# Lukeasargen/Show-Attend-and-Tell-Pytorch-Lightning

Hardware: AMD Instinct MI355X
Metric: captions/sec (train step) at B=128, 256px, seq_len=22 (higher is better)
Workload: dtype bf16; 1 GPU; C2: resnet50 encoder_size=7 encoder_dim=512 vocab=6400 T=22, 128 images/GPU x R=5 captions, trainable encoder, Adam, full lengths, decoder_tf=always; global_batch_images=128, parallelism=dp1, grad_bucket_dtype=fp32

## Files before the change

### show-attend-and-tell-pytorch-lightning_amd/csrc/api.hip

```cpp
#include <stdarg.h>

#include "../../include/sat_hip.h"
#include "decoder.h"
#include "decoder_step.h"
#include "gemm.h"
#include "gemm_bf16_common.h"
#include "temperature.h"
#include "caption_score.h"

namespace sat {
static thread_local char g_err[512] = {0};
int& dev_switch(int which) {
    static int v[SW_COUNT] = {0 , getenv("SAT_NO_WGRAD3X3") ? !atoi(getenv("SAT_NO_WGRAD3X3")) : 1,
                              getenv("SAT_REDUCE_Z16") ? atoi(getenv("SAT_REDUCE_Z16")) : 1, getenv("SAT_WIDE_TILES") ? atoi(getenv("SAT_WIDE_TILES")) : 0,
                              getenv("SAT_BN_ONEPASS") ? atoi(getenv("SAT_BN_ONEPASS")) : 1,
                              getenv("SAT_BN_VPT") ? atoi(getenv("SAT_BN_VPT")) : 2,
                              getenv("SAT_ACC_PREFETCH") ? atoi(getenv("SAT_ACC_PREFETCH")) : 0};
    return v[which];
}
int& trace_launches() { static int on = getenv("SAT_TRACE_LAUNCH") ? 1 : 0; return on; }
char* last_error_buf() { return g_err; }
int fail(int code, const char* fmt, ...) {
    va_list ap; va_start(ap, fmt); vsnprintf(g_err, sizeof g_err, fmt, ap); va_end(ap);
    return code;
}
}

using namespace sat;

extern "C" {

int sat_abi_version(void) { return SAT_HIP_ABI_VERSION; }
int sat_debug_trace_launches(int32_t on) { sat::trace_launches() = on ? 1 : 0; return SAT_OK; }
int sat_debug_option(const char* name, int32_t value) {
    if (!name) return fail(SAT_EINVAL, "debug_option: null name");
    if (!strcmp(name, "wgrad3x3")) { dev_switch(SW_WGRAD3X3) = value; return SAT_OK; }
    if (!strcmp(name, "reduce_z16")) { dev_switch(SW_REDUCE_Z16) = value; return SAT_OK; }
    if (!strcmp(name, "acc_prefetch")) { dev_switch(SW_ACC_PREFETCH) = value; return SAT_OK; }
    if (!strcmp(name, "bn_vpt")) { dev_switch(SW_BN_VPT) = value; return SAT_OK; }
    if (!strcmp(name, "bn_onepass")) { dev_switch(SW_BN_ONEPASS) = value; return SAT_OK; }
    if (!strcmp(name, "wide_tiles")) { dev_switch(SW_WIDE_TILES) = value; return SAT_OK; }
    if (!strcmp(name, "glds_tile")) { glds_force_tile() = value; return SAT_OK; }
    if (!strcmp(name, "glds_stages8")) { glds_stages8() = value; return SAT_OK; }
    if (!strcmp(name, "glds_tall_k")) { glds_tall_k() = value; return SAT_OK; }
    if (!strcmp(name, "glds_tall_conv")) { glds_tall_conv() = value; return SAT_OK; }
    if (!strcmp(name, "tile_override")) { gemm_tile_override() = value; return SAT_OK; }
    return fail(SAT_EINVAL, "debug_option: unknown option %s", name);
}
const char* sat_last_error(void) { return last_error_buf(); }

static int gemm_from_desc(const sat_gemm_desc* d, const sat_gemm_types* t, void* stream);
int sat_gemm_f32(const sat_gemm_desc* d, void* stream) { return gemm_from_desc(d, nullptr, stream); }
int sat_gemm_ex(const sat_gemm_desc* d, const sat_gemm_types* t, void* stream) {
    if (!t) return fail(SAT_EINVAL, "sat_gemm_ex: null type descriptor");
    return gemm_from_desc(d, t, stream);
}
static int gemm_from_desc(const sat_gemm_desc* d, const sat_gemm_types* t, void* stream) {
    if (!d) return fail(SAT_EINVAL, "sat_gemm_f32: null descriptor");
    if (d->amode != A_ROW && d->amode != A_KMAJOR) return fail(SAT_EINVAL, "sat_gemm_f32: amode %d (dense modes only)", d->amode);
    if (d->bmode != B_ROW && d->bmode != B_KMAJOR) return fail(SAT_EINVAL, "sat_gemm_f32: bmode %d (dense modes only)", d->bmode);
    GemmArgs g;
    g.A = d->A; g.lda = d->lda; g.a_rows = d->a_rows; g.B = d->B; g.ldb = d->ldb; g.C = d->C; g.ldc = d->ldc; g.c_rows = d->c_rows;
    g.M = d->M; g.N = d->N; g.K = d->K; g.amode = d->amode; g.bmode = d->bmode; g.accumulate = d->accumulate; g.epi = d->epi;
    g.bias = d->bias; g.e0 = d->e0; g.lde0 = d->lde0; g.c0 = d->c0; g.c1 = d->c1; g.slab = d->slab; g.slab_elems = d->slab_elems;
    if (t) { g.a_bf16 = t->a_bf16; g.b_bf16 = t->b_bf16; g.c_bf16 = t->c_bf16; g.bf16_mfma = t->bf16_mfma; }
    return launch_gemm(g, (hipStream_t)stream);
}

size_t sat_decoder_workspace_bytes(const sat_decoder_dims* d) {
    if (check_dims(d) != SAT_OK) return 0;
    return decoder_workspace_bytes(*d);
}

size_t sat_decoder_workspace_bytes_ln(const sat_decoder_dims* d, const sat_decoder_params* w) {
    if (check_dims(d) != SAT_OK) return 0;
    return decoder_workspace_bytes(*d, w && ln_on(*w));
}

static int check_params(const sat_decoder_dims* d, const sat_decoder_params* w, const char* what) {
    if (!w) return fail(SAT_EINVAL, "%s: null parameter struct", what);
    if (!w->embedding || !w->init_f_w || !w->init_f_b || !w->init_i_w || !w->init_i_b || !w->w_ih || !w->w_hh || !w->b_ih || !w->b_hh ||
        !w->att_enc || !w->att_dec || !w->att_f || !w->beta_w || !w->beta_b || !w->out_hidden || !w->out_w)
        return fail(SAT_EINVAL, "%s: null tensor in parameter struct", what);
    if (d->deep_output && !w->out_context) return fail(SAT_EINVAL, "%s: deep output needs output.context.weight", what);
    for (int l = 1; l < d->layers; ++l)
        if (!w->up_w_ih[l - 1] || !w->up_w_hh[l - 1] || !w->up_b_ih[l - 1] || !w->up_b_hh[l - 1])
            return fail(SAT_EINVAL, "%s: null tensor for LSTM layer %d", what, l);
    int ln_set = 0;
    for (int l = 0; l < d->layers; ++l) ln_set += (w->ln_gate_w[l] != nullptr) + (w->ln_gate_b[l] != nullptr) + (w->ln_cell_w[l] != nullptr) + (w->ln_cell_b[l] != nullptr);
    if (ln_set != 0 && ln_set != 4 * d->layers)
        return fail(SAT_EINVAL, "%s: %d of the %d layer-norm tensors (ln_gate_w / ln_gate_b / ln_cell_w / ln_cell_b of %d layers) are set: all or none", what, ln_set,
                    4 * d->layers, d->layers);
    return SAT_OK;
}
static int check_batch(const sat_decoder_batch* b) {
// ... 648 lines not shown
```

### show-attend-and-tell-pytorch-lightning_amd/csrc/gemm_bf16_common.h

```cpp
#pragma once
#include <stdlib.h>

#include "gemm.h"

namespace sat {

typedef __bf16 bf16x8 __attribute__((ext_vector_type(8)));
typedef __bf16 bf16x4 __attribute__((ext_vector_type(4)));
typedef short s16x4 __attribute__((ext_vector_type(4)));
typedef float f32x16 __attribute__((ext_vector_type(16)));

constexpr int NT = 256;

struct BArgs {
    const void* A; long lda; const int* a_rows;
    const void* B; long ldb;
    void* C; long ldc; const int* c_rows;
    int M, N, K;
    int accumulate, epi;
    const float* bias; const float* e0; long lde0; int c0, c1;
    ConvGeom g;
    int kchunk, nsplit;
    float* slab;
    int wide_store;
// ... 423 lines not shown
}

template <typename TC>
__global__ __launch_bounds__(256) void splitk_reduce_z16_kernel(BArgs a) {
    __shared__ float4 part[16][16];
    const int ev = threadIdx.x & 15, zl = threadIdx.x >> 4;
    const long idx4 = (long)blockIdx.x * 16 + ev;
    const long total4 = (long)a.M * a.N / 4;
    float4 v = make_float4(0.f, 0.f, 0.f, 0.f);
    if (idx4 < total4) {
        const float4* s4 = reinterpret_cast<const float4*>(a.slab);
#pragma unroll 4
        for (int z = zl; z < a.nsplit; z += 16) { const float4 t = s4[(long)z * total4 + idx4]; v.x += t.x; v.y += t.y; v.z += t.z; v.w += t.w; }
    }
    part[zl][ev] = v;
    __syncthreads();
    if (zl != 0 || idx4 >= total4) return;
#pragma unroll
    for (int l = 1; l < 16; ++l) { const float4 t = part[l][ev]; v.x += t.x; v.y += t.y; v.z += t.z; v.w += t.w; }
    const long e = idx4 * 4; const int row = (int)(e / a.N), col = (int)(e % a.N);
    if (sizeof(TC) == 4 && a.wide_store && !a.g.cls) {
        float* dst = reinterpret_cast<float*>(a.C) + (long)row * a.ldc + col;
        if (a.accumulate) { const float4 old = *reinterpret_cast<const float4*>(dst); v.x += old.x; v.y += old.y; v.z += old.z; v.w += old.w; }
        if (a.epi != EPI_NONE) { v.x = ep_value(a, row, col, v.x); v.y = ep_value(a, row, col + 1, v.y); v.z = ep_value(a, row, col + 2, v.z); v.w = ep_value(a, row, col + 3, v.w); }
        *reinterpret_cast<float4*>(dst) = v;
    } else {
        put<TC>(a, row, col, v.x); put<TC>(a, row, col + 1, v.y); put<TC>(a, row, col + 2, v.z); put<TC>(a, row, col + 3, v.w);
    }
}

template <typename TC>
inline int launch_splitk_reduce(const BArgs& k, hipStream_t st) {
    const long total = (long)k.M * k.N;
    const int z16 = dev_switch(SW_REDUCE_Z16);
    if (k.wide_slab && z16 && k.nsplit >= 32 && total / 4 / 256 < 256)
        hipLaunchKernelGGL(splitk_reduce_z16_kernel<TC>, dim3(cdiv(total / 4, 16)), dim3(256), 0, st, k);
    else if (k.wide_slab) hipLaunchKernelGGL(splitk_reduce_b4_kernel<TC>, dim3(cdiv(total / 4, 256)), dim3(256), 0, st, k);
    else hipLaunchKernelGGL(splitk_reduce_b_kernel<TC>, dim3(cdiv(total, 256)), dim3(256), 0, st, k);
    return launch_ok("splitk_reduce_b");
}

__device__ __forceinline__ void xcd_tile(int& bx, int& by, int& bz, int y_fastest = 0) {
    const unsigned total = gridDim.x * gridDim.y * gridDim.z;
    const unsigned orig = (blockIdx.z * gridDim.y + blockIdx.y) * gridDim.x + blockIdx.x;
    const unsigned q = total >> 3, r = total & 7, xcd = orig & 7, idx = orig >> 3;
    const unsigned lin = (xcd < r ? xcd * (q + 1) : r * (q + 1) + (xcd - r) * q) + idx;
    if (y_fastest) { by = lin % gridDim.y; const unsigned t2 = lin / gridDim.y; bx = t2 % gridDim.x; bz = t2 / gridDim.x; }
    else { bx = lin % gridDim.x; const unsigned t2 = lin / gridDim.x; by = t2 % gridDim.y; bz = t2 / gridDim.y; }
}

int launch_gemm_glds(const BArgs& k, int amode, int bmode, int c_bf16, int BMt, hipStream_t st, int* bm_used = nullptr);
int& glds_force_tile();
int& glds_stages8();
int& glds_tall_k();
int& glds_tall_conv();
int& glds_ablate();
int& gemm_tile_override();

}
```

### show-attend-and-tell-pytorch-lightning_amd/csrc/gemm_glds.hip

```cpp
#include <stdlib.h>

#include "gemm_bf16_common.h"

namespace sat {

template <int AM, int BMo, typename TC> int glds_run_64(const BArgs& k, hipStream_t st);
template <int AM, int BMo, typename TC> int glds_run_128(const BArgs& k, hipStream_t st);
template <int AM, int BMo, typename TC> int glds_run_128x64(const BArgs& k, hipStream_t st);
#ifdef SAT_DEV_TILES
template <int AM, int BMo, typename TC> int glds_run_256x128(const BArgs& k, hipStream_t st);
template <int AM, int BMo, typename TC> int glds_run_256(const BArgs& k, hipStream_t st);
#endif

enum { TILE_64 = 0, TILE_128 = 1, TILE_128x64 = 2, TILE_256x128 = 3, TILE_256 = 4 };
template <int AM, int BMo, typename TC>
static int rung_tiles(const BArgs& k, int tile, hipStream_t st, int* bm_used) {
    switch (tile) {
#ifdef SAT_DEV_TILES
        case TILE_256: if (bm_used) *bm_used = 256; return glds_run_256<AM, BMo, TC>(k, st);
        case TILE_256x128: if (bm_used) *bm_used = 256; return glds_run_256x128<AM, BMo, TC>(k, st);
#else
        case TILE_256: case TILE_256x128: return -1;
#endif
        case TILE_128: if (bm_used) *bm_used = 128; return glds_run_128<AM, BMo, TC>(k, st);
        case TILE_128x64: if (bm_used) *bm_used = 128; return glds_run_128x64<AM, BMo, TC>(k, st);
        default: if (bm_used) *bm_used = 64; return glds_run_64<AM, BMo, TC>(k, st);
    }
}

int& glds_force_tile() { static int v = getenv("SAT_GLDS_TILE") ? atoi(getenv("SAT_GLDS_TILE")) : -1; return v; }
int& glds_ablate() { static int v = 0; return v; }
int& glds_tall_k() { static int v = getenv("SAT_GLDS_TALL_K") ? atoi(getenv("SAT_GLDS_TALL_K")) : 1 << 30; return v; }
int& glds_tall_conv() { static int v = getenv("SAT_GLDS_TALL_CONV") ? atoi(getenv("SAT_GLDS_TALL_CONV")) : 1152; return v; }
int& glds_stages8() { static int v = getenv("SAT_GLDS_STAGES8") ? atoi(getenv("SAT_GLDS_STAGES8")) : 0; return v; }

int launch_gemm_glds(const BArgs& k0, int amode, int bmode, int c_bf16, int BMt, hipStream_t st, int* bm_used) {
    const int force_tile = glds_force_tile();
    static const int off = getenv("SAT_NO_GLDS") ? atoi(getenv("SAT_NO_GLDS")) : 0;
    static const int force_stages = getenv("SAT_GLDS_STAGES") ? atoi(getenv("SAT_GLDS_STAGES")) : 0;
    static const int deep_from = getenv("SAT_GLDS_DEEP_FROM") ? atoi(getenv("SAT_GLDS_DEEP_FROM")) : 1 << 30;
    static const int rotate = getenv("SAT_GLDS_ROT") ? atoi(getenv("SAT_GLDS_ROT")) : 1 << 20;
    if (off) return -1;
    BArgs k = k0;
    const int ktiles = cdiv(k.kchunk < k.K ? k.kchunk : k.K, 64);
    static const int s1_upto = getenv("SAT_GLDS_S1_UPTO") ? atoi(getenv("SAT_GLDS_S1_UPTO")) : 1 << 30;
    k.nstage = force_stages ? force_stages : (ktiles >= deep_from ? 4 : ((ktiles == 1 || (c_bf16 && ktiles <= s1_upto)) ? 1 : 2));
    k.rotate = rotate;
    if (k.nstage < 1) k.nstage = 1;
    if (k.nstage > 4) k.nstage = 4;
    static const int tall = getenv("SAT_GLDS_TALL") ? atoi(getenv("SAT_GLDS_TALL")) : 2;
    int tile = (BMt >= 256) ? (BMt == 256 ? TILE_256 : TILE_256x128) : (BMt == 128 ? TILE_128 : TILE_64);
    if (tile == TILE_64 && tall && bmode != B_CONV_WGRAD && k.N <= 64 && (amode == A_KMAJOR ? (tall > 1 && k.M >= 128) : k.M >= 8192)) tile = TILE_128x64;
    static const int tall_conv_tiles = getenv("SAT_GLDS_TALL_CONV_TILES") ? atoi(getenv("SAT_GLDS_TALL_CONV_TILES")) : 512;
    if (tile == TILE_128 && bmode != B_CONV_WGRAD && k.nsplit <= 1 &&
        ((amode == A_ROW && k.K <= glds_tall_k()) || ((amode == A_CONV_FWD || amode == A_CONV_DGRAD) && (k.K <= glds_tall_conv() || (long)cdiv(k.M, 128) * cdiv(k.N, 128) < tall_conv_tiles)))) tile = TILE_128x64;
    if (force_tile >= 0) tile = force_tile;
    if (tile == TILE_256 || tile == TILE_256x128) {
        const int maxs = (tile == TILE_256) ? 2 : 3;
        const int deep8 = glds_stages8();
        if (ktiles > 1) k.nstage = deep8 ? (deep8 < maxs ? deep8 : maxs) : (ktiles >= 3 ? maxs : 2);
    }
    {
        static const int order = getenv("SAT_TILE_ORDER") ? atoi(getenv("SAT_TILE_ORDER")) : -1;
        const int tbm = (tile == TILE_64) ? 64 : 128, tbn = (tile == TILE_128) ? 128 : 64;
        const int mt = cdiv(k.M, tbm), nt = cdiv(k.N, tbn);
        k.y_fastest = order >= 0 ? order : (amode == A_ROW && bmode != B_CONV_WGRAD && mt <= 16 && nt >= 2 * mt);
    }
    const ConvGeom& g = k.g;
    if (g.sw && g.sw != g.stride) return -1;
    if (k.K % 64 || k.kchunk % 64 || k.a_rows) return -1;
    if (amode == A_CONV_FWD && (g.C % 64 || g.R * g.S > 32)) return -1;
    if (amode == A_CONV_DGRAD && (g.K % 64 || g.R * g.S > 32 || (g.stride != 1 && !g.cls))) return -1;
    if (bmode == B_CONV_WGRAD && g.R * g.S > 32) return -1;
    const long lim = 1L << 30;
    long a_el = 0, b_el = 0;
    switch (amode) {
        case A_ROW: a_el = (long)k.M * k.lda; break;
        case A_KMAJOR: a_el = (long)k.K * k.lda; break;
        case A_CONV_FWD: a_el = (long)g.N * g.H * g.W * g.C; break;
        default: a_el = (long)g.N * g.P * g.Q * g.K; break;
    }
    switch (bmode) {
        case B_ROW: b_el = (long)k.N * k.ldb; break;
        case B_KMAJOR: b_el = (long)k.K * k.ldb; break;
        case B_CONV_WGRAD: b_el = (long)g.N * g.H * g.W * g.C; break;
        default: b_el = (long)g.K * g.R * g.S * g.C; break;
    }
    if (a_el >= lim || b_el >= lim) return -1;
    if ((amode == A_KMAJOR && k.M < 8) || (bmode != B_ROW && k.N < 8)) return -1;
#define SAT_GCASE(AMV, BMV, TC) return rung_tiles<AMV, BMV, TC>(k, tile, st, bm_used);
    if (amode == A_CONV_FWD && bmode == B_ROW && c_bf16) SAT_GCASE(A_CONV_FWD, B_ROW, __bf16)
    if (amode == A_ROW && bmode == B_ROW && c_bf16) SAT_GCASE(A_ROW, B_ROW, __bf16)
    if (amode == A_ROW && bmode == B_ROW && !c_bf16) SAT_GCASE(A_ROW, B_ROW, float)
    if (amode == A_CONV_DGRAD && bmode == B_CONV_DGRAD_W && c_bf16) SAT_GCASE(A_CONV_DGRAD, B_CONV_DGRAD_W, __bf16)
    if (amode == A_ROW && bmode == B_KMAJOR && c_bf16) SAT_GCASE(A_ROW, B_KMAJOR, __bf16)
    if (amode == A_ROW && bmode == B_KMAJOR && !c_bf16) SAT_GCASE(A_ROW, B_KMAJOR, float)
    if (amode == A_KMAJOR && bmode == B_CONV_WGRAD && !c_bf16) SAT_GCASE(A_KMAJOR, B_CONV_WGRAD, float)
    if (amode == A_KMAJOR && bmode == B_KMAJOR && !c_bf16) SAT_GCASE(A_KMAJOR, B_KMAJOR, float)
#undef SAT_GCASE
// ... 5 lines not shown
```

### show-attend-and-tell-pytorch-lightning_amd/csrc/gemm_glds_kernel.h

```cpp
#include <stdlib.h>

#include <initializer_list>

#pragma once
#include "gemm_bf16_common.h"
#include "profile.h"

#ifndef SAT_GLDS_ABLATE
#define SAT_GLDS_ABLATE 0
#endif

namespace sat {

typedef int i32x4 __attribute__((ext_vector_type(4)));
typedef __attribute__((address_space(3))) void* lptr_t;

__device__ void raw_buffer_load_lds(i32x4 rsrc, lptr_t lds, int size, int voffset, int soffset, int offset, int aux) __asm("llvm.amdgcn.raw.buffer.load.lds");

constexpr int OOB = (int)0x80000000;

__device__ __forceinline__ i32x4 make_rsrc(const void* base) {
    const unsigned long long b = reinterpret_cast<unsigned long long>(base);
    i32x4 r;
    r[0] = (int)(unsigned)b; r[1] = (int)(unsigned)((b >> 32) & 0xFFFF);
    r[2] = OOB;
    r[3] = 0x00020000;
    return r;
}
__device__ __forceinline__ void dma16(const i32x4& rsrc, int voff, int soff, __bf16* lds_wave_base) {
    raw_buffer_load_lds(rsrc, (lptr_t)lds_wave_base, 16, voff, soff, 0, 0);
}

__device__ __forceinline__ unsigned bit_range(int lo, int hi) {
    if (lo < 0) lo = 0;
    if (hi > 32) hi = 32;
    if (hi <= lo) return 0u;
    const unsigned upper = (hi >= 32) ? 0xFFFFFFFFu : ((1u << hi) - 1u);
    return upper & ~((1u << lo) - 1u);
}
__device__ __forceinline__ unsigned tap_mask(int rlo, int rhi, int clo, int chi, int nrow, int ncol) {
    const unsigned cm = bit_range(clo, chi < ncol ? chi : ncol);
    unsigned m = 0;
    if (rlo < 0) rlo = 0;
    if (rhi > nrow) rhi = nrow;
    for (int i = rlo; i < rhi; ++i) m |= cm << (i * ncol);
    return m;
}

template <typename T> __device__ __forceinline__ void keep_alive(const T& v) {
#if defined(__HIP_DEVICE_COMPILE__)
    asm volatile("" ::"v"(v));
#endif
}
template <typename T, typename U> __device__ __forceinline__ void keep_alive(const T& v, const U& w) { keep_alive(v); keep_alive(w); }

struct PixEnt { int off; unsigned mask; };

#ifndef SAT_GLDS_BN_PREFETCH
// ... 180 lines not shown

    f32x16 acc[TM][TN];
#pragma unroll
    for (int i = 0; i < TM; ++i)
#pragma unroll
        for (int j = 0; j < TN; ++j)
#pragma unroll
            for (int r = 0; r < 16; ++r) acc[i][j][r] = 0.f;

    constexpr bool BNS = (AM == A_CONV_DGRAD) || (AM == A_ROW && BMo == B_KMAJOR);
    constexpr bool BPF = SAT_GLDS_BN_PREFETCH;
    BnAcc<BM, BN, 64 * NW, BNS, BPF> bnacc(a, bn, tid);
    if constexpr (sizeof(TC) == 2) { bnacc.prefetch(a, bm, bn, tid); __builtin_amdgcn_sched_barrier(0); }

    int a_off[TM], a_sw[TM], b_off[TN], b_sw[TN];
#pragma unroll
    for (int i = 0; i < TM; ++i) {
        if (!AK) { const int row = wm + i * 32 + li; a_off[i] = row * KB; a_sw[i] = (row >> 1) & 7; }
        else {
            const int col = wm + i * 32 + 16 * t_mh + 4 * t_p, kr = 8 * t_h + t_q;
            const int sw = (BM >= 128) ? (kr & 3) : ((kr >> 1) & 1);
            a_off[i] = kr * BM + (((col >> 5) ^ sw) << 5) + (col & 31); a_sw[i] = 0;
        }
    }
#pragma unroll
    for (int j = 0; j < TN; ++j) {
        if (!BKM) { const int row = wn + j * 32 + li; b_off[j] = row * KB; b_sw[j] = (row >> 1) & 7; }
        else {
            const int col = wn + j * 32 + 16 * t_mh + 4 * t_p, kr = 8 * t_h + t_q;
            const int sw = (BN >= 128) ? (kr & 3) : ((kr >> 1) & 1);
            b_off[j] = kr * BN + (((col >> 5) ^ sw) << 5) + (col & 31); b_sw[j] = 0;
        }
    }

    if (kbeg < kend) {
        if (WG) {
            for (int t = 0; t < S; ++t) fill_tab(t, t);
            __syncthreads();
        }
        const int pre = (S == 1) ? 1 : S - 1;
        for (int t = 0; t < pre && t < T; ++t) issue(t, t);
        int cur = 0, nxt = S - 1;
        for (int it = 0; it < T; ++it) {
            const int ahead = (S == 1) ? 0 : min(T - 1 - it, S - 2);
            if (ahead >= 2) asm volatile("s_waitcnt vmcnt(%0)" ::"n"(2 * G) : "memory");
            else if (ahead == 1) asm volatile("s_waitcnt vmcnt(%0)" ::"n"(G) : "memory");
            else asm volatile("s_waitcnt vmcnt(0)" ::: "memory");
            asm volatile("s_waitcnt lgkmcnt(0)" ::: "memory");
            __builtin_amdgcn_s_barrier();
            asm volatile("" ::: "memory");
            const bool more = S > 1 && it + S - 1 < T;
            const __bf16* as = smem + cur * STAGE;
            const __bf16* bs = as + A_EL;
            bf16x8 af[2][TM], bf[2][TN];
            auto load_frags = [&](int kk, bf16x8 (&fa)[TM], bf16x8 (&fb)[TN]) {
#pragma unroll
                for (int i = 0; i < TM; ++i) {
                    if (!AK) fa[i] = *reinterpret_cast<const bf16x8*>(as + a_off[i] + ((((kk >> 3) + lh) ^ a_sw[i]) << 3));
                    else {
                        const __bf16* p = as + a_off[i] + kk * BM;
                        bf16x4 lo = __builtin_amdgcn_ds_read_tr16_b64_v4bf16((__attribute__((address_space(3))) bf16x4*)p);
                        bf16x4 hi = __builtin_amdgcn_ds_read_tr16_b64_v4bf16((__attribute__((address_space(3))) bf16x4*)(p + 4 * BM));
                        fa[i] = __builtin_shufflevector(lo, hi, 0, 1, 2, 3, 4, 5, 6, 7);
                    }
                }
#pragma unroll
                for (int j = 0; j < TN; ++j) {
                    if (!BKM) fb[j] = *reinterpret_cast<const bf16x8*>(bs + b_off[j] + ((((kk >> 3) + lh) ^ b_sw[j]) << 3));
                    else {
                        const __bf16* p = bs + b_off[j] + kk * BN;
                        bf16x4 lo = __builtin_amdgcn_ds_read_tr16_b64_v4bf16((__attribute__((address_space(3))) bf16x4*)p);
                        bf16x4 hi = __builtin_amdgcn_ds_read_tr16_b64_v4bf16((__attribute__((address_space(3))) bf16x4*)(p + 4 * BN));
                        fb[j] = __builtin_shufflevector(lo, hi, 0, 1, 2, 3, 4, 5, 6, 7);
                    }
                }
            };
            if (!(abl & 4) || it == 0) load_frags(0, af[0], bf[0]);
#pragma unroll
            for (int ks = 0; ks < KB / 16; ++ks) {
                if (ks + 1 < KB / 16 && (!(abl & 4) || it == 0)) load_frags((ks + 1) * 16, af[(ks + 1) & 1], bf[(ks + 1) & 1]);
                if (more) {
#pragma unroll
                    for (int jj = (ks * G) / 4; jj < ((ks + 1) * G) / 4; ++jj) issue_piece(nxt, nxt, jj);
                }
                if constexpr (!(abl & 2)) {
#pragma unroll
                    for (int i = 0; i < TM; ++i)
#pragma unroll
                        for (int j = 0; j < TN; ++j)
                            acc[i][j] = __builtin_amdgcn_mfma_f32_32x32x16_bf16(af[ks & 1][i], bf[ks & 1][j], acc[i][j], 0, 0, 0);
                } else {
#pragma unroll
                    for (int i = 0; i < TM; ++i)
#pragma unroll
                        for (int j = 0; j < TN; ++j) keep_alive(af[ks & 1][i], bf[ks & 1][j]);
                }
            }
            if (more) advance_tile();
            if (S == 1 && it + 1 < T) {
                __syncthreads();
                if (WG) { fill_tab(0, it + 1); __syncthreads(); }
                issue(0, 0);
            }
            if (WG && S > 1) fill_tab(cur, it + S);
            cur = (cur + 1 == S) ? 0 : cur + 1;
            nxt = (nxt + 1 == S) ? 0 : nxt + 1;
        }
    }
    if constexpr (abl & 8) {
#pragma unroll
        for (int i = 0; i < TM; ++i)
#pragma unroll
            for (int j = 0; j < TN; ++j) keep_alive(acc[i][j]);
        return;
    }
    if constexpr (WR == 2 && WC == 2) store_tile<BM, BN, TC, 2 * STAGE, APF, BNS, BPF>(a, acc, smem, bm, bn, bz, wm, wn, tid, lane, bnacc, sizeof(TC) == 2);
    else store_tile_w<BM, BN, WR, WC, TC, BNS, BPF>(a, acc, smem, bm, bn, bz, wm, wn, wrow, tid, lane, bnacc, sizeof(TC) == 2);
}

static const char* gname(int am, int bm) {
    if (am == A_CONV_FWD) return "conv_fwd";
    if (am == A_CONV_DGRAD) return "conv_dgrad";
    if (bm == B_CONV_WGRAD) return "conv_wgrad";
    if (am == A_ROW && bm == B_ROW) return "nt";
    if (am == A_ROW && bm == B_KMAJOR) return "nn";
    return "tn";
}

template <int BM, int BN, int WR, int WC, int AM, int BMo, typename TC>
static int rung(const BArgs& k, hipStream_t st) {
    dim3 grid(cdiv(k.N, BN), cdiv(k.M, BM), k.nsplit);
    char pname[128];
    if (profile_enabled()) {
        static const bool shapes = getenv("SAT_PROFILE_SHAPES") != nullptr;
        if (shapes) snprintf(pname, sizeof pname, "gemm_glds_%s_%dx%d M%d N%d K%d z%d", gname(AM, BMo), BM, BN, k.M, k.N, k.K, k.nsplit);
        else snprintf(pname, sizeof pname, "gemm_glds_%s_%dx%d", gname(AM, BMo), BM, BN);
    }
    ProfScope prof(pname, 2.0 * k.M * k.N * k.K, 2.0 * k.M * k.K + 2.0 * k.N * k.K + (double)sizeof(TC) * k.M * k.N, st);
    size_t lds = (size_t)k.nstage * (BM + BN) * 64 * sizeof(__bf16);
    const size_t epi_lds = (WR == 2 && WC == 2) ? ((sizeof(TC) == 2) ? (size_t)BM * (BN + 8) * 2 + 4 * BN * 2 * 4 : (size_t)(BM / 2) * (BN + 4) * 4)
                                                : store_lds_bytes<BM, BN, WR, WC, TC>();
    if (lds < epi_lds) lds = epi_lds;
    constexpr size_t LDS_DYN_MAX = 160 * 1024 - 2560;
    SAT_REQUIRE(lds <= LDS_DYN_MAX, "gemm_glds: %zu bytes of LDS for a %dx%d tile with %d stages", lds, BM, BN, k.nstage);
    static bool attr_set = false;
    if (!attr_set) {
        SAT_CHECK_HIP(hipFuncSetAttribute(reinterpret_cast<const void*>(&gemm_glds_kernel<BM, BN, WR, WC, AM, BMo, TC>), hipFuncAttributeMaxDynamicSharedMemorySize,
                                          (int)LDS_DYN_MAX));
// ... 38 lines not shown
```

### show-attend-and-tell-pytorch-lightning_amd/csrc/wgrad3x3.hip

```cpp
#include <stdlib.h>

#include "gemm_bf16_common.h"
#include "profile.h"

namespace sat {

typedef int i32x4 __attribute__((ext_vector_type(4)));
typedef __attribute__((address_space(3))) void* lptr3_t;
__device__ void raw_buffer_load_lds_w(i32x4 rsrc, lptr3_t lds, int size, int voffset, int soffset, int offset, int aux) __asm("llvm.amdgcn.raw.buffer.load.lds");

namespace {
constexpr int W3_OOB = (int)0x80000000;
constexpr int W3_WAVES = 9, W3_THREADS = 64 * W3_WAVES;
constexpr int W3_MAXP = 4;
constexpr int W3_STAGES = 3;

__device__ __forceinline__ i32x4 w3_rsrc(const void* base) {
    const unsigned long long b = reinterpret_cast<unsigned long long>(base);
    i32x4 r;
    r[0] = (int)(unsigned)b; r[1] = (int)(unsigned)((b >> 32) & 0xFFFF);
    r[2] = W3_OOB; r[3] = 0x00020000;
    return r;
}

struct W3Args {
    const __bf16* dy; const __bf16* x; float* out;
    int Nimg, H, W, C, K;
    int nr;
    int units;
    int per;
    int HP;
    int Z;
};

__global__ __launch_bounds__(W3_THREADS) void wgrad3x3_kernel(W3Args a) {
    extern __shared__ __attribute__((aligned(1024))) __bf16 smem[];
    const int tid = threadIdx.x, lane = tid & 63, wave = tid >> 6;
    const int ci0 = blockIdx.x * 64, co0 = blockIdx.y * 64, bz = blockIdx.z;
    const int W = a.W, H = a.H, C = a.C, K = a.K, nr = a.nr, HW2 = W + 2;
    const int STAGE = 64 * 64 + a.HP * 64;
    const int u0 = bz * a.per, u1 = min(a.units, u0 + a.per);
    const int upi = H / nr;
    const i32x4 rA = w3_rsrc(a.dy), rX = w3_rsrc(a.x);

    const int npieces = 8 + a.HP / 8;
    int p_off[W3_MAXP]; int p_hr[W3_MAXP]; bool p_dy[W3_MAXP], p_on[W3_MAXP], p_colok[W3_MAXP]; int p_lds[W3_MAXP];
#pragma unroll
    for (int j = 0; j < W3_MAXP; ++j) {
        const int piece = j * W3_WAVES + wave;
        p_on[j] = piece < npieces; p_dy[j] = piece < 8; p_hr[j] = 0; p_colok[j] = false; p_off[j] = 0;
        const int sl = lane & 7;
        if (p_dy[j]) {
            const int krow = piece * 8 + (lane >> 3);
            const int lq = (sl >> 2) ^ ((krow >> 1) & 1);
            p_off[j] = (krow * K + co0 + (lq * 4 + (sl & 3)) * 8) * 2;
            p_lds[j] = piece * 512;
        } else {
            const int hp = (piece - 8) * 8 + (lane >> 3);
            const int hr = hp / HW2, hc = hp - hr * HW2 - 1;
            const int lq = (sl >> 2) ^ ((hp >> 1) & 1);
            p_hr[j] = hr;
            p_colok[j] = p_on[j] && hr < nr + 2 && hc >= 0 && hc < W;
            p_off[j] = ((hr * W + hc) * C + ci0 + (lq * 4 + (sl & 3)) * 8) * 2;
            p_lds[j] = 64 * 64 + (piece - 8) * 512;
        }
    }
    auto issue = [&](int buf, int u) {
        const int n = u / upi, p0 = (u - n * upi) * nr;
        const int baseA = ((n * H + p0) * W) * K * 2;
        const int baseX = ((n * H + p0 - 1) * W) * C * 2;
        __bf16* st = smem + buf * STAGE;
#pragma unroll
        for (int j = 0; j < W3_MAXP; ++j) {
            if (!p_on[j]) continue;
            if (p_dy[j]) raw_buffer_load_lds_w(rA, (lptr3_t)(st + p_lds[j]), 16, p_off[j] + baseA, 0, 0, 0);
            else {
                const int ih = p0 - 1 + p_hr[j];
                const bool ok = p_colok[j] && ih >= 0 && ih < H;
                raw_buffer_load_lds_w(rX, (lptr3_t)(st + p_lds[j]), 16, ok ? p_off[j] + baseX : W3_OOB, 0, 0, 0);
            }
        }
    };

    const int tg = lane >> 4, ti = lane & 15;
    const int t_h = tg >> 1, t_mh = tg & 1, t_q = ti >> 2, t_p = ti & 3;
    const int tap_r = wave / 3, tap_s = wave - tap_r * 3;
    int a_off[2];
#pragma unroll
    for (int i = 0; i < 2; ++i) {
        const int col = i * 32 + 16 * t_mh + 4 * t_p, kr = 8 * t_h + t_q;
        a_off[i] = kr * 64 + (((col >> 5) ^ ((kr >> 1) & 1)) << 5) + (col & 31);
    }
    int b_off[4][2][2];
#pragma unroll
    for (int ks = 0; ks < 4; ++ks)
#pragma unroll
        for (int hf = 0; hf < 2; ++hf) {
            const int k = ks * 16 + 8 * t_h + t_q + 4 * hf;
            const int pr = k / W, q = k - pr * W;
            const int hp = (pr + tap_r) * HW2 + q + tap_s;
#pragma unroll
            for (int j = 0; j < 2; ++j) {
                const int col = j * 32 + 16 * t_mh + 4 * t_p;
                b_off[ks][hf][j] = 64 * 64 + hp * 64 + (((col >> 5) ^ ((hp >> 1) & 1)) << 5) + (col & 31);
            }
        }

    f32x16 acc[2][2];
#pragma unroll
    for (int i = 0; i < 2; ++i)
#pragma unroll
        for (int j = 0; j < 2; ++j)
#pragma unroll
            for (int r = 0; r < 16; ++r) acc[i][j][r] = 0.f;

    int mine = 0;
#pragma unroll
    for (int j = 0; j < W3_MAXP; ++j) mine += p_on[j] ? 1 : 0;
    mine = __builtin_amdgcn_readfirstlane(mine);
    if (u0 < u1) {
        issue(0, u0);
        if (u0 + 1 < u1) issue(1, u0 + 1);
        int cur = 0, nxt = 2;
        for (int u = u0; u < u1; ++u) {
            if (u + 1 < u1) {
                if (mine == 4) asm volatile("s_waitcnt vmcnt(4)" ::: "memory");
                else if (mine == 3) asm volatile("s_waitcnt vmcnt(3)" ::: "memory");
                else if (mine == 2) asm volatile("s_waitcnt vmcnt(2)" ::: "memory");
                else asm volatile("s_waitcnt vmcnt(0)" ::: "memory");
            } else asm volatile("s_waitcnt vmcnt(0)" ::: "memory");
            asm volatile("s_waitcnt lgkmcnt(0)" ::: "memory");
            __builtin_amdgcn_s_barrier();
            asm volatile("" ::: "memory");
            if (u + 2 < u1) issue(nxt, u + 2);
            const __bf16* st = smem + cur * STAGE;
#pragma unroll
            for (int ks = 0; ks < 4; ++ks) {
                bf16x8 af[2], bf[2];
#pragma unroll
                for (int i = 0; i < 2; ++i) {
                    const __bf16* p = st + a_off[i] + ks * 16 * 64;
                    bf16x4 lo = __builtin_amdgcn_ds_read_tr16_b64_v4bf16((__attribute__((address_space(3))) bf16x4*)p);
                    bf16x4 hi = __builtin_amdgcn_ds_read_tr16_b64_v4bf16((__attribute__((address_space(3))) bf16x4*)(p + 4 * 64));
                    af[i] = __builtin_shufflevector(lo, hi, 0, 1, 2, 3, 4, 5, 6, 7);
                }
#pragma unroll
                for (int j = 0; j < 2; ++j) {
                    bf16x4 lo = __builtin_amdgcn_ds_read_tr16_b64_v4bf16((__attribute__((address_space(3))) bf16x4*)(st + b_off[ks][0][j]));
                    bf16x4 hi = __builtin_amdgcn_ds_read_tr16_b64_v4bf16((__attribute__((address_space(3))) bf16x4*)(st + b_off[ks][1][j]));
                    bf[j] = __builtin_shufflevector(lo, hi, 0, 1, 2, 3, 4, 5, 6, 7);
                }
#pragma unroll
                for (int i = 0; i < 2; ++i)
#pragma unroll
                    for (int j = 0; j < 2; ++j) acc[i][j] = __builtin_amdgcn_mfma_f32_32x32x16_bf16(af[i], bf[j], acc[i][j], 0, 0, 0);
            }
            cur = (cur + 1 == W3_STAGES) ? 0 : cur + 1;
            nxt = (nxt + 1 == W3_STAGES) ? 0 : nxt + 1;
        }
    }
    const int li = lane & 31, lh = lane >> 5;
    const long N9 = 9L * C;
    float* out = a.out + (a.Z > 1 ? (long)bz * K * N9 : 0L);
#pragma unroll
    for (int i = 0; i < 2; ++i)
#pragma unroll
        for (int j = 0; j < 2; ++j)
#pragma unroll
            for (int r = 0; r < 16; ++r) {
                const int row = co0 + i * 32 + (r & 3) + 8 * (r >> 2) + 4 * lh;
                const int col = ci0 + j * 32 + li;
                out[(long)row * N9 + (long)wave * C + col] = acc[i][j][r];
            }
}
}

int wgrad3x3_eligible(const ConvGeom& g) {
    if (!dev_switch(SW_WGRAD3X3)) return 0;
    if (g.R != 3 || g.S != 3 || g.stride != 1 || g.pad != 1 || (g.sw && g.sw != 1)) return 0;
    if (g.C % 64 || g.K % 64) return 0;
    if (g.H != g.P || g.W != g.Q) return 0;
    if (!(g.W == 8 || g.W == 16 || g.W == 32 || g.W == 64)) return 0;
    if (g.H % (64 / g.W)) return 0;
    if ((long)g.N * g.H * g.W * (g.C > g.K ? g.C : g.K) >= (1L << 30)) return 0;
    return 1;
}

int launch_wgrad3x3(const void* dy, const void* x, float* dw, const ConvGeom& g, float* slab, long slab_elems, hipStream_t st) {
    W3Args a;
    a.dy = reinterpret_cast<const __bf16*>(dy); a.x = reinterpret_cast<const __bf16*>(x);
    a.Nimg = g.N; a.H = g.H; a.W = g.W; a.C = g.C; a.K = g.K;
    a.nr = 64 / g.W; a.units = g.N * (g.H / a.nr);
    a.HP = ((a.nr + 2) * (g.W + 2) + 7) / 8 * 8;
    SAT_REQUIRE(8 + a.HP / 8 <= W3_WAVES * W3_MAXP, "wgrad3x3: %d LDS-DMA pieces per k-tile", 8 + a.HP / 8);
    const long tiles = (long)(g.C / 64) * (g.K / 64), out_elems = (long)g.K * 9 * g.C;
    static const int target = getenv("SAT_W3_TARGET") ? atoi(getenv("SAT_W3_TARGET")) : 256;
    long z = target / tiles; if (z < 1) z = 1;
    if (z > a.units / 8) z = a.units / 8 > 0 ? a.units / 8 : 1;
    while (z > 1 && (!slab || z * out_elems > slab_elems)) --z;
    a.per = (int)cdiv(a.units, z); a.Z = (int)cdiv(a.units, a.per);
    a.out = a.Z > 1 ? slab : dw;
    const size_t lds = W3_STAGES * (size_t)(64 * 64 + a.HP * 64) * sizeof(__bf16);
    static bool attr_set = false;
    if (!attr_set) {
        SAT_CHECK_HIP(hipFuncSetAttribute(reinterpret_cast<const void*>(&wgrad3x3_kernel), hipFuncAttributeMaxDynamicSharedMemorySize, 128 * 1024));
        attr_set = true;
    }
    {
        char pname[128];
        if (profile_enabled()) {
            static const bool shapes = getenv("SAT_PROFILE_SHAPES") != nullptr;
            if (shapes) snprintf(pname, sizeof pname, "gemm_wgrad3x3 M%d N%d K%d z%d", g.K, 9 * g.C, g.N * g.H * g.W, a.Z);
            else snprintf(pname, sizeof pname, "gemm_wgrad3x3");
        }
        ProfScope prof(pname, 2.0 * g.K * 9.0 * g.C * g.N * g.H * g.W, 2.0 * g.N * g.H * g.W * ((double)g.C + g.K) + 4.0 * out_elems, st);
        hipLaunchKernelGGL(wgrad3x3_kernel, dim3(g.C / 64, g.K / 64, a.Z), dim3(W3_THREADS), lds, st, a);
        SAT_TRY(launch_ok("wgrad3x3_kernel"));
        if (a.Z > 1) {
            BArgs k{};
            k.M = g.K; k.N = 9 * g.C; k.C = dw; k.ldc = 9 * g.C; k.slab = slab; k.nsplit = a.Z; k.wide_store = 1; k.wide_slab = 1; k.epi = EPI_NONE;
            SAT_TRY(launch_splitk_reduce<float>(k, st));
        }
    }
    return SAT_OK;
}

}
```

Before: 32570 captions/s.

## Use inline-asm LDS fragment reads with partial lgkmcnt waits and tunable stage counts

```diff
diff --git a/show-attend-and-tell-pytorch-lightning_amd/csrc/api.hip b/show-attend-and-tell-pytorch-lightning_amd/csrc/api.hip
--- a/show-attend-and-tell-pytorch-lightning_amd/csrc/api.hip
+++ b/show-attend-and-tell-pytorch-lightning_amd/csrc/api.hip
@@ -41,6 +41,10 @@
     if (!strcmp(name, "bn_onepass")) { dev_switch(SW_BN_ONEPASS) = value; return SAT_OK; }
     if (!strcmp(name, "wide_tiles")) { dev_switch(SW_WIDE_TILES) = value; return SAT_OK; }
     if (!strcmp(name, "glds_tile")) { glds_force_tile() = value; return SAT_OK; }
+    if (!strcmp(name, "glds_stages")) { glds_force_stages() = value; return SAT_OK; }
+    if (!strcmp(name, "glds_stages_tr_bf16")) { glds_stages_tr_bf16() = value; return SAT_OK; }
+    if (!strcmp(name, "glds_stages_f32")) { glds_stages_f32() = value; return SAT_OK; }
+    if (!strcmp(name, "w3_stages")) { w3_stages() = value; return SAT_OK; }
     if (!strcmp(name, "glds_stages8")) { glds_stages8() = value; return SAT_OK; }
     if (!strcmp(name, "glds_tall_k")) { glds_tall_k() = value; return SAT_OK; }
     if (!strcmp(name, "glds_tall_conv")) { glds_tall_conv() = value; return SAT_OK; }
diff --git a/show-attend-and-tell-pytorch-lightning_amd/csrc/gemm_bf16_common.h b/show-attend-and-tell-pytorch-lightning_amd/csrc/gemm_bf16_common.h
--- a/show-attend-and-tell-pytorch-lightning_amd/csrc/gemm_bf16_common.h
+++ b/show-attend-and-tell-pytorch-lightning_amd/csrc/gemm_bf16_common.h
@@ -499,6 +499,10 @@
 int launch_gemm_glds(const BArgs& k, int amode, int bmode, int c_bf16, int BMt, hipStream_t st, int* bm_used = nullptr);
 int& glds_force_tile();
 int& glds_stages8();
+int& glds_stages_tr_bf16();
+int& glds_stages_f32();
+int& w3_stages();
+int& glds_force_stages();
 int& glds_tall_k();
 int& glds_tall_conv();
 int& glds_ablate();
diff --git a/show-attend-and-tell-pytorch-lightning_amd/csrc/gemm_glds.hip b/show-attend-and-tell-pytorch-lightning_amd/csrc/gemm_glds.hip
--- a/show-attend-and-tell-pytorch-lightning_amd/csrc/gemm_glds.hip
+++ b/show-attend-and-tell-pytorch-lightning_amd/csrc/gemm_glds.hip
@@ -30,6 +30,9 @@
 
 int& glds_force_tile() { static int v = getenv("SAT_GLDS_TILE") ? atoi(getenv("SAT_GLDS_TILE")) : -1; return v; }
 int& glds_ablate() { static int v = 0; return v; }
+int& glds_stages_tr_bf16() { static int v = getenv("SAT_GLDS_STAGES_TR_BF16") ? atoi(getenv("SAT_GLDS_STAGES_TR_BF16")) : 1; return v; }
+int& glds_stages_f32() { static int v = getenv("SAT_GLDS_STAGES_F32") ? atoi(getenv("SAT_GLDS_STAGES_F32")) : 2; return v; }
+int& glds_force_stages() { static int v = getenv("SAT_GLDS_STAGES") ? atoi(getenv("SAT_GLDS_STAGES")) : 0; return v; }
 int& glds_tall_k() { static int v = getenv("SAT_GLDS_TALL_K") ? atoi(getenv("SAT_GLDS_TALL_K")) : 1 << 30; return v; }
 int& glds_tall_conv() { static int v = getenv("SAT_GLDS_TALL_CONV") ? atoi(getenv("SAT_GLDS_TALL_CONV")) : 1152; return v; }
 int& glds_stages8() { static int v = getenv("SAT_GLDS_STAGES8") ? atoi(getenv("SAT_GLDS_STAGES8")) : 0; return v; }
@@ -37,14 +40,14 @@
 int launch_gemm_glds(const BArgs& k0, int amode, int bmode, int c_bf16, int BMt, hipStream_t st, int* bm_used) {
     const int force_tile = glds_force_tile();
     static const int off = getenv("SAT_NO_GLDS") ? atoi(getenv("SAT_NO_GLDS")) : 0;
-    static const int force_stages = getenv("SAT_GLDS_STAGES") ? atoi(getenv("SAT_GLDS_STAGES")) : 0;
+    const int force_stages = glds_force_stages();
     static const int deep_from = getenv("SAT_GLDS_DEEP_FROM") ? atoi(getenv("SAT_GLDS_DEEP_FROM")) : 1 << 30;
     static const int rotate = getenv("SAT_GLDS_ROT") ? atoi(getenv("SAT_GLDS_ROT")) : 1 << 20;
     if (off) return -1;
     BArgs k = k0;
     const int ktiles = cdiv(k.kchunk < k.K ? k.kchunk : k.K, 64);
-    static const int s1_upto = getenv("SAT_GLDS_S1_UPTO") ? atoi(getenv("SAT_GLDS_S1_UPTO")) : 1 << 30;
-    k.nstage = force_stages ? force_stages : (ktiles >= deep_from ? 4 : ((ktiles == 1 || (c_bf16 && ktiles <= s1_upto)) ? 1 : 2));
+    const int by_form = c_bf16 ? (bmode != B_ROW ? glds_stages_tr_bf16() : 1) : glds_stages_f32();
+    k.nstage = force_stages ? force_stages : (ktiles >= deep_from ? 4 : (ktiles == 1 ? 1 : by_form));
     k.rotate = rotate;
     if (k.nstage < 1) k.nstage = 1;
     if (k.nstage > 4) k.nstage = 4;
diff --git a/show-attend-and-tell-pytorch-lightning_amd/csrc/gemm_glds_kernel.h b/show-attend-and-tell-pytorch-lightning_amd/csrc/gemm_glds_kernel.h
--- a/show-attend-and-tell-pytorch-lightning_amd/csrc/gemm_glds_kernel.h
+++ b/show-attend-and-tell-pytorch-lightning_amd/csrc/gemm_glds_kernel.h
@@ -1,9 +1,11 @@
 #include <stdlib.h>
 
 #include <initializer_list>
+#include <type_traits>
 
 #pragma once
 #include "gemm_bf16_common.h"
+#include "lds_frag.h"
 #include "profile.h"
 
 #ifndef SAT_GLDS_ABLATE
@@ -290,48 +292,86 @@
             const bool more = S > 1 && it + S - 1 < T;
             const __bf16* as = smem + cur * STAGE;
             const __bf16* bs = as + A_EL;
-            bf16x8 af[2][TM], bf[2][TN];
-            auto load_frags = [&](int kk, bf16x8 (&fa)[TM], bf16x8 (&fb)[TN]) {
-#pragma unroll
-                for (int i = 0; i < TM; ++i) {
-                    if (!AK) fa[i] = *reinterpret_cast<const bf16x8*>(as + a_off[i] + ((((kk >> 3) + lh) ^ a_sw[i]) << 3));
-                    else {
-                        const __bf16* p = as + a_off[i] + kk * BM;
-                        bf16x4 lo = __builtin_amdgcn_ds_read_tr16_b64_v4bf16((__attribute__((address_space(3))) bf16x4*)p);
-                        bf16x4 hi = __builtin_amdgcn_ds_read_tr16_b64_v4bf16((__attribute__((address_space(3))) bf16x4*)(p + 4 * BM));
-                        fa[i] = __builtin_shufflevector(lo, hi, 0, 1, 2, 3, 4, 5, 6, 7);
-                    }
-                }
-#pragma unroll
-                for (int j = 0; j < TN; ++j) {
-                    if (!BKM) fb[j] = *reinterpret_cast<const bf16x8*>(bs + b_off[j] + ((((kk >> 3) + lh) ^ b_sw[j]) << 3));
-                    else {
-                        const __bf16* p = bs + b_off[j] + kk * BN;
-                        bf16x4 lo = __builtin_amdgcn_ds_read_tr16_b64_v4bf16((__attribute__((address_space(3))) bf16x4*)p);
-                        bf16x4 hi = __builtin_amdgcn_ds_read_tr16_b64_v4bf16((__attribute__((address_space(3))) bf16x4*)(p + 4 * BN));
-                        fb[j] = __builtin_shufflevector(lo, hi, 0, 1, 2, 3, 4, 5, 6, 7);
-                    }
-                }
-            };
-            if (!(abl & 4) || it == 0) load_frags(0, af[0], bf[0]);
-#pragma unroll
-            for (int ks = 0; ks < KB / 16; ++ks) {
-                if (ks + 1 < KB / 16 && (!(abl & 4) || it == 0)) load_frags((ks + 1) * 16, af[(ks + 1) & 1], bf[(ks + 1) & 1]);
-                if (more) {
-#pragma unroll
-                    for (int jj = (ks * G) / 4; jj < ((ks + 1) * G) / 4; ++jj) issue_piece(nxt, nxt, jj);
-                }
-                if constexpr (!(abl & 2)) {
+            if constexpr (AK || BKM) {
+                constexpr int RD = (AK ? 2 : 1) * TM + (BKM ? 2 : 1) * TN;
+                constexpr int A_B = A_EL * 2;
+                static_assert(A_B + (48 + 4) * BN * 2 < 65536 && (48 + 4) * BM * 2 < 65536, "fragment offsets must fit the ds offset field");
+                const unsigned sbase = lds_addr(smem) + (unsigned)(cur * (STAGE * 2));
+                unsigned a_ad[TM], b_ad[TN];
+#pragma unroll
+                for (int i = 0; i < TM; ++i) a_ad[i] = sbase + a_off[i] * 2;
+#pragma unroll
+                for (int j = 0; j < TN; ++j) b_ad[j] = sbase + b_off[j] * 2;
+                Frag fa[2][TM], fb[2][TN];
+                auto read_frags = [&](auto kc, Frag (&xa)[TM], Frag (&xb)[TN]) {
+                    constexpr int kk = decltype(kc)::value;
+#pragma unroll
+                    for (int i = 0; i < TM; ++i) {
+                        if constexpr (AK) { xa[i].lo = lds_read_tr16<kk * BM * 2>(a_ad[i]); xa[i].hi = lds_read_tr16<(kk + 4) * BM * 2>(a_ad[i]); }
+                        else xa[i].q = lds_read_b128<0>(a_ad[i] + (((((kk >> 3) + lh) ^ a_sw[i]) << 3) * 2));
+                    }
+#pragma unroll
+                    for (int j = 0; j < TN; ++j) {
+                        if constexpr (BKM) { xb[j].lo = lds_read_tr16<A_B + kk * BN * 2>(b_ad[j]); xb[j].hi = lds_read_tr16<A_B + (kk + 4) * BN * 2>(b_ad[j]); }
+                        else xb[j].q = lds_read_b128<A_B>(b_ad[j] + (((((kk >> 3) + lh) ^ b_sw[j]) << 3) * 2));
+                    }
+                };
+                auto k_step = [&](auto kc) {
+                    constexpr int ks = decltype(kc)::value;
+                    constexpr bool ahead = ks + 1 < KB / 16;
+                    if constexpr (ahead) {
+                        if (!(abl & 4) || it == 0) read_frags(std::integral_constant<int, (ks + 1) * 16>{}, fa[(ks + 1) & 1], fb[(ks + 1) & 1]);
+                    }
+                    if (more) {
+#pragma unroll
+                        for (int jj = (ks * G) / 4; jj < ((ks + 1) * G) / 4; ++jj) issue_piece(nxt, nxt, jj);
+                    }
+                    lds_wait<ahead ? (RD < 15 ? RD : 15) : 0>();
+                    bf16x8 va[TM], vb[TN];
+#pragma unroll
+                    for (int i = 0; i < TM; ++i) { frag_landed<AK>(fa[ks & 1][i]); va[i] = frag_value<AK>(fa[ks & 1][i]); }
+#pragma unroll
+                    for (int j = 0; j < TN; ++j) { frag_landed<BKM>(fb[ks & 1][j]); vb[j] = frag_value<BKM>(fb[ks & 1][j]); }
 #pragma unroll
                     for (int i = 0; i < TM; ++i)
 #pragma unroll
-                        for (int j = 0; j < TN; ++j)
-                            acc[i][j] = __builtin_amdgcn_mfma_f32_32x32x16_bf16(af[ks & 1][i], bf[ks & 1][j], acc[i][j], 0, 0, 0);
-                } else {
-#pragma unroll
-                    for (int i = 0; i < TM; ++i)
-#pragma unroll
-                        for (int j = 0; j < TN; ++j) keep_alive(af[ks & 1][i], bf[ks & 1][j]);
+                        for (int j = 0; j < TN; ++j) {
+                            if constexpr (!(abl & 2)) acc[i][j] = __builtin_amdgcn_mfma_f32_32x32x16_bf16(va[i], vb[j], acc[i][j], 0, 0, 0);
+                            else keep_alive(va[i], vb[j]);
+                        }
+                };
+                if (!(abl & 4) || it == 0) read_frags(std::integral_constant<int, 0>{}, fa[0], fb[0]);
+                static_assert(KB / 16 == 4, "four k-steps per tile");
+                k_step(std::integral_constant<int, 0>{}); k_step(std::integral_constant<int, 1>{});
+                k_step(std::integral_constant<int, 2>{}); k_step(std::integral_constant<int, 3>{});
+            } else {
+                bf16x8 af[2][TM], bf[2][TN];
+                auto load_frags = [&](int kk, bf16x8 (&fa)[TM], bf16x8 (&fb)[TN]) {
+#pragma unroll
+                    for (int i = 0; i < TM; ++i) fa[i] = *reinterpret_cast<const bf16x8*>(as + a_off[i] + ((((kk >> 3) + lh) ^ a_sw[i]) << 3));
+#pragma unroll
+                    for (int j = 0; j < TN; ++j) fb[j] = *reinterpret_cast<const bf16x8*>(bs + b_off[j] + ((((kk >> 3) + lh) ^ b_sw[j]) << 3));
+                };
+                if (!(abl & 4) || it == 0) load_frags(0, af[0], bf[0]);
+#pragma unroll
+                for (int ks = 0; ks < KB / 16; ++ks) {
+                    if (ks + 1 < KB / 16 && (!(abl & 4) || it == 0)) load_frags((ks + 1) * 16, af[(ks + 1) & 1], bf[(ks + 1) & 1]);
+                    if (more) {
+#pragma unroll
+                        for (int jj = (ks * G) / 4; jj < ((ks + 1) * G) / 4; ++jj) issue_piece(nxt, nxt, jj);
+                    }
+                    if constexpr (!(abl & 2)) {
+#pragma unroll
+                        for (int i = 0; i < TM; ++i)
+#pragma unroll
+                            for (int j = 0; j < TN; ++j)
+                                acc[i][j] = __builtin_amdgcn_mfma_f32_32x32x16_bf16(af[ks & 1][i], bf[ks & 1][j], acc[i][j], 0, 0, 0);
+                    } else {
+#pragma unroll
+                        for (int i = 0; i < TM; ++i)
+#pragma unroll
+                            for (int j = 0; j < TN; ++j) keep_alive(af[ks & 1][i], bf[ks & 1][j]);
+                    }
                 }
             }
             if (more) advance_tile();
diff --git a/show-attend-and-tell-pytorch-lightning_amd/csrc/lds_frag.h b/show-attend-and-tell-pytorch-lightning_amd/csrc/lds_frag.h
--- /dev/null
+++ b/show-attend-and-tell-pytorch-lightning_amd/csrc/lds_frag.h
@@ -0,0 +1,45 @@
+#pragma once
+#include "gemm_bf16_common.h"
+
+namespace sat {
+
+typedef int i32x4 __attribute__((ext_vector_type(4)));
+
+typedef int i32x2 __attribute__((ext_vector_type(2)));
+struct Frag { i32x2 lo, hi; i32x4 q; };
+
+__device__ __forceinline__ unsigned lds_addr(const __bf16* p) {
+    return (unsigned)(size_t)(__attribute__((address_space(3))) const __bf16*)p;
+}
+template <int OFF> __device__ __forceinline__ i32x2 lds_read_tr16(unsigned addr) {
+    static_assert(OFF >= 0 && OFF < 65536, "ds offset field");
+    i32x2 v = {0, 0};
+#if defined(__HIP_DEVICE_COMPILE__)
+    asm volatile("ds_read_b64_tr_b16 %0, %1 offset:%2" : "=v"(v) : "v"(addr), "n"(OFF) : "memory");
+#endif
+    return v;
+}
+template <int OFF> __device__ __forceinline__ i32x4 lds_read_b128(unsigned addr) {
+    static_assert(OFF >= 0 && OFF < 65536, "ds offset field");
+    i32x4 v = {0, 0, 0, 0};
+#if defined(__HIP_DEVICE_COMPILE__)
+    asm volatile("ds_read_b128 %0, %1 offset:%2" : "=v"(v) : "v"(addr), "n"(OFF) : "memory");
+#endif
+    return v;
+}
+template <int N> __device__ __forceinline__ void lds_wait() {
+    static_assert(N >= 0 && N <= 15, "lgkmcnt field");
+    asm volatile("s_waitcnt lgkmcnt(%0)" ::"n"(N) : "memory");
+}
+template <bool TR> __device__ __forceinline__ void frag_landed(Frag& f) {
+#if defined(__HIP_DEVICE_COMPILE__)
+    if constexpr (TR) asm volatile("" : "+v"(f.lo), "+v"(f.hi));
+    else asm volatile("" : "+v"(f.q));
+#endif
+}
+template <bool TR> __device__ __forceinline__ bf16x8 frag_value(const Frag& f) {
+    if constexpr (TR) return __builtin_bit_cast(bf16x8, __builtin_shufflevector(f.lo, f.hi, 0, 1, 2, 3));
+    else return __builtin_bit_cast(bf16x8, f.q);
+}
+
+}
diff --git a/show-attend-and-tell-pytorch-lightning_amd/csrc/wgrad3x3.hip b/show-attend-and-tell-pytorch-lightning_amd/csrc/wgrad3x3.hip
--- a/show-attend-and-tell-pytorch-lightning_amd/csrc/wgrad3x3.hip
+++ b/show-attend-and-tell-pytorch-lightning_amd/csrc/wgrad3x3.hip
@@ -1,6 +1,9 @@
 #include <stdlib.h>
 
+#include <type_traits>
+
 #include "gemm_bf16_common.h"
+#include "lds_frag.h"
 #include "profile.h"
 
 namespace sat {
@@ -14,6 +17,7 @@
 constexpr int W3_WAVES = 9, W3_THREADS = 64 * W3_WAVES;
 constexpr int W3_MAXP = 4;
 constexpr int W3_STAGES = 3;
+constexpr int W3_MIN_STAGES = 2, W3_MAX_STAGES = 4;
 
 __device__ __forceinline__ i32x4 w3_rsrc(const void* base) {
     const unsigned long long b = reinterpret_cast<unsigned long long>(base);
@@ -31,6 +35,7 @@
     int per;
     int HP;
     int Z;
+    int S;
 };
 
 __global__ __launch_bounds__(W3_THREADS) void wgrad3x3_kernel(W3Args a) {
@@ -118,45 +123,58 @@
 #pragma unroll
     for (int j = 0; j < W3_MAXP; ++j) mine += p_on[j] ? 1 : 0;
     mine = __builtin_amdgcn_readfirstlane(mine);
+    const int S = a.S;
     if (u0 < u1) {
-        issue(0, u0);
-        if (u0 + 1 < u1) issue(1, u0 + 1);
-        int cur = 0, nxt = 2;
+        for (int t = 0; t < S - 1 && u0 + t < u1; ++t) issue(t, u0 + t);
+        int cur = 0, nxt = S - 1;
         for (int u = u0; u < u1; ++u) {
-            if (u + 1 < u1) {
-                if (mine == 4) asm volatile("s_waitcnt vmcnt(4)" ::: "memory");
-                else if (mine == 3) asm volatile("s_waitcnt vmcnt(3)" ::: "memory");
-                else if (mine == 2) asm volatile("s_waitcnt vmcnt(2)" ::: "memory");
-                else asm volatile("s_waitcnt vmcnt(0)" ::: "memory");
-            } else asm volatile("s_waitcnt vmcnt(0)" ::: "memory");
+            const int ahead = min(u1 - 1 - u, S - 2);
+            switch (mine * ahead) {
+                case 2: asm volatile("s_waitcnt vmcnt(2)" ::: "memory"); break;
+                case 3: asm volatile("s_waitcnt vmcnt(3)" ::: "memory"); break;
+                case 4: asm volatile("s_waitcnt vmcnt(4)" ::: "memory"); break;
+                case 6: asm volatile("s_waitcnt vmcnt(6)" ::: "memory"); break;
+                case 8: asm volatile("s_waitcnt vmcnt(8)" ::: "memory"); break;
+                default: asm volatile("s_waitcnt vmcnt(0)" ::: "memory"); break;
+            }
             asm volatile("s_waitcnt lgkmcnt(0)" ::: "memory");
             __builtin_amdgcn_s_barrier();
             asm volatile("" ::: "memory");
-            if (u + 2 < u1) issue(nxt, u + 2);
-            const __bf16* st = smem + cur * STAGE;
-#pragma unroll
-            for (int ks = 0; ks < 4; ++ks) {
+            if (u + S - 1 < u1) issue(nxt, u + S - 1);
+            const unsigned sbase = lds_addr(smem) + (unsigned)(cur * STAGE * 2);
+            Frag fa[2][2], fb[2][2];
+            auto read_frags = [&](auto kc, Frag (&xa)[2], Frag (&xb)[2]) {
+                constexpr int ks = decltype(kc)::value;
+#pragma unroll
+                for (int i = 0; i < 2; ++i) {
+                    xa[i].lo = lds_read_tr16<ks * 16 * 64 * 2>(sbase + a_off[i] * 2);
+                    xa[i].hi = lds_read_tr16<(ks * 16 + 4) * 64 * 2>(sbase + a_off[i] * 2);
+                }
+#pragma unroll
+                for (int j = 0; j < 2; ++j) {
+                    xb[j].lo = lds_read_tr16<0>(sbase + b_off[ks][0][j] * 2);
+                    xb[j].hi = lds_read_tr16<0>(sbase + b_off[ks][1][j] * 2);
+                }
+            };
+            auto k_step = [&](auto kc) {
+                constexpr int ks = decltype(kc)::value;
+                if constexpr (ks + 1 < 4) read_frags(std::integral_constant<int, ks + 1>{}, fa[(ks + 1) & 1], fb[(ks + 1) & 1]);
+                lds_wait<(ks + 1 < 4) ? 8 : 0>();
                 bf16x8 af[2], bf[2];
 #pragma unroll
-                for (int i = 0; i < 2; ++i) {
-                    const __bf16* p = st + a_off[i] + ks * 16 * 64;
-                    bf16x4 lo = __builtin_amdgcn_ds_read_tr16_b64_v4bf16((__attribute__((address_space(3))) bf16x4*)p);
-                    bf16x4 hi = __builtin_amdgcn_ds_read_tr16_b64_v4bf16((__attribute__((address_space(3))) bf16x4*)(p + 4 * 64));
-                    af[i] = __builtin_shufflevector(lo, hi, 0, 1, 2, 3, 4, 5, 6, 7);
-                }
-#pragma unroll
-                for (int j = 0; j < 2; ++j) {
-                    bf16x4 lo = __builtin_amdgcn_ds_read_tr16_b64_v4bf16((__attribute__((address_space(3))) bf16x4*)(st + b_off[ks][0][j]));
-                    bf16x4 hi = __builtin_amdgcn_ds_read_tr16_b64_v4bf16((__attribute__((address_space(3))) bf16x4*)(st + b_off[ks][1][j]));
-                    bf[j] = __builtin_shufflevector(lo, hi, 0, 1, 2, 3, 4, 5, 6, 7);
-                }
+                for (int i = 0; i < 2; ++i) { frag_landed<true>(fa[ks & 1][i]); af[i] = frag_value<true>(fa[ks & 1][i]); }
+#pragma unroll
+                for (int j = 0; j < 2; ++j) { frag_landed<true>(fb[ks & 1][j]); bf[j] = frag_value<true>(fb[ks & 1][j]); }
 #pragma unroll
                 for (int i = 0; i < 2; ++i)
 #pragma unroll
                     for (int j = 0; j < 2; ++j) acc[i][j] = __builtin_amdgcn_mfma_f32_32x32x16_bf16(af[i], bf[j], acc[i][j], 0, 0, 0);
-            }
-            cur = (cur + 1 == W3_STAGES) ? 0 : cur + 1;
-            nxt = (nxt + 1 == W3_STAGES) ? 0 : nxt + 1;
+            };
+            read_frags(std::integral_constant<int, 0>{}, fa[0], fb[0]);
+            k_step(std::integral_constant<int, 0>{}); k_step(std::integral_constant<int, 1>{});
+            k_step(std::integral_constant<int, 2>{}); k_step(std::integral_constant<int, 3>{});
+            cur = (cur + 1 == S) ? 0 : cur + 1;
+            nxt = (nxt + 1 == S) ? 0 : nxt + 1;
         }
     }
     const int li = lane & 31, lh = lane >> 5;
@@ -174,6 +192,8 @@
             }
 }
 }
+
+int& w3_stages() { static int v = getenv("SAT_W3_STAGES") ? atoi(getenv("SAT_W3_STAGES")) : W3_STAGES; return v; }
 
 int wgrad3x3_eligible(const ConvGeom& g) {
     if (!dev_switch(SW_WGRAD3X3)) return 0;
@@ -200,10 +220,13 @@
     while (z > 1 && (!slab || z * out_elems > slab_elems)) --z;
     a.per = (int)cdiv(a.units, z); a.Z = (int)cdiv(a.units, a.per);
     a.out = a.Z > 1 ? slab : dw;
-    const size_t lds = W3_STAGES * (size_t)(64 * 64 + a.HP * 64) * sizeof(__bf16);
+    const int forced = glds_force_stages();
+    const int want = forced ? forced : w3_stages();
+    a.S = want < W3_MIN_STAGES ? W3_MIN_STAGES : (want > W3_MAX_STAGES ? W3_MAX_STAGES : want);
+    const size_t lds = a.S * (size_t)(64 * 64 + a.HP * 64) * sizeof(__bf16);
     static bool attr_set = false;
     if (!attr_set) {
-        SAT_CHECK_HIP(hipFuncSetAttribute(reinterpret_cast<const void*>(&wgrad3x3_kernel), hipFuncAttributeMaxDynamicSharedMemorySize, 128 * 1024));
+        SAT_CHECK_HIP(hipFuncSetAttribute(reinterpret_cast<const void*>(&wgrad3x3_kernel), hipFuncAttributeMaxDynamicSharedMemorySize, 144 * 1024));
         attr_set = true;
     }
     {
```

Result: faster. 32920 captions/s, median of 6 (+1.1%).
